# AIGC-Audio/AudioGPT

Measured on NVIDIA H100. Metric: mel_frames_per_s_vocoded, higher is better.
Workload: dtype f32

## Files before the change

audiogpt_b200/csrc/hifigan.cu:

```cuda
#include "common.cuh"
#include "tapconv.cuh"
#include "models.h"
#include "voc_kernels.cuh"

namespace agpt {

__global__ void cf_to_cl_kernel(const float* __restrict__ in, float* __restrict__ out, int C, int T) {
  __shared__ float tile[32][33];
  const int b = blockIdx.z, t0 = blockIdx.x * 32, c0 = blockIdx.y * 32;
  const float* ib = in + (long)b * C * T;
  float* ob = out + (long)b * C * T;
  for (int i = threadIdx.y; i < 32; i += blockDim.y) {
    const int c = c0 + i, t = t0 + threadIdx.x;
    tile[i][threadIdx.x] = (c < C && t < T) ? ib[(long)c * T + t] : 0.f;
  }
  __syncthreads();
  for (int i = threadIdx.y; i < 32; i += blockDim.y) {
    const int t = t0 + i, c = c0 + threadIdx.x;
    if (t < T && c < C) ob[(long)t * C + c] = tile[threadIdx.x][i];
  }
}

void launch_cf_to_cl(const float* in, float* out, int B, int C, int T, cudaStream_t st) {
  dim3 grid(cdiv(T, 32), cdiv(C, 32), B), block(32, 8);
// ... 239 lines not shown
    double inc = run;
#pragma unroll
    for (int o = 1; o < 32; o <<= 1) { const double v = __shfl_up_sync(0xffffffffu, inc, o); if (lane >= o) inc += v; }
    __syncthreads();
    if (lane == 31) wsum[warp] = inc;
    __syncthreads();
    double base = cbase[((long)b * dim + h) * nch + c];
    for (int w = 0; w < warp; ++w) base += wsum[w];
    base += inc - run;
#pragma unroll
    for (int k = 0; k < 4; ++k) {
      const int t = t0 + k;
      if (t >= L) continue;
      double ph = base + r[k];
      ph -= floor(ph);
      const float sn = sinf((float)ph * 6.283185307179586f) * sine_amp;
      const float uv = fv[k] > thr ? 1.f : 0.f;
      const float na = uv * noise_std + (1.f - uv) * sine_amp / 3.f;
      const float nz = noise ? noise[((long)b * L + t) * dim + h] : 0.f;
      acc[k] = fmaf(lin.w[h], sn * uv + na * nz, acc[k]);
    }
  }
#pragma unroll
  for (int k = 0; k < 4; ++k)
    if (t0 + k < L) har[(long)b * L + t0 + k] = tanhf(acc[k]);
}

static DevBuf g_nsf_scratch[16];

void nsf_source(const float* f0, int B, int L, int dim, float sr, const float* lin_w_host, float lin_b,
                const float* rand_ini, const float* noise, float sine_amp, float noise_std, float thr, float* har,
                cudaStream_t st) {
  AGPT_CHECK(B >= 1 && L >= 1 && dim >= 1 && dim <= NSF_MAXH, "nsf_source: bad shape (at most 16 harmonics)");
  int dev = 0;
  AGPT_CUDA(cudaGetDevice(&dev));
  const int nch = cdiv(L, NSF_CHUNK);
  double* cs = reinterpret_cast<double*>(g_nsf_scratch[dev & 15].ensure((size_t)B * dim * nch * 2 + 2));
  NsfLin lin;
  for (int h = 0; h < NSF_MAXH; ++h) lin.w[h] = h < dim ? lin_w_host[h] : 0.f;
  lin.b = lin_b;
  nsf_chunk_sum_kernel<<<dim3(nch, dim, B), 256, 0, st>>>(f0, cs, L, dim, sr);
  nsf_chunk_scan_kernel<<<cdiv(B * dim, 64), 64, 0, st>>>(cs, rand_ini, nch, dim, B);
  nsf_source_kernel<<<dim3(nch, B), 256, 0, st>>>(f0, cs, noise, har, L, dim, sr, sine_amp, noise_std, thr, lin);
  count_launch(3);
  AGPT_CUDA(cudaGetLastError());
}

struct SnakeW { DevBuf a, inv_b; };

struct ResBlockW {
  int ks = 0;
  std::vector<int> dil;
  std::vector<PackedConv> c1, c2;
  std::vector<PackedConv> c1g, c2g;
  std::vector<int> g1, g2;
  std::vector<SnakeW> act;
};

struct NoiseConvW {
  DevBuf w, b;
  int K = 0, st = 1, pad = 0, C = 0;
};

struct Hifigan : Handle {
  agpt_hifigan_cfg cfg;
  PackedConv conv_pre;
  std::vector<PackedConv> ups;
  std::vector<ResBlockW> rbs;
  std::vector<NoiseConvW> noise;
  DevBuf post_w, post_b;
  SnakeW act_post;
  AaFilter aaf;
  int c_last = 0, hop = 1;
  DevBuf melT, buf[6], sbuf;
  DevBuf plane[6];
  DevBuf io_mel, io_wav, io_har;
  float* pin_mel = nullptr; float* pin_wav = nullptr; size_t pin_mel_n = 0, pin_wav_n = 0;
  cudaStream_t own_stream = nullptr;
  bool fuse_resblock = true;
  bool tall_tiles = true;
  bool plane_feed = true;
  bool pair_dual = true;
  bool pair_pipe = true;
  bool narrow_pipe = true;
  bool conv_pipe = true;

  ~Hifigan() override {
    if (pin_mel) cudaFreeHost(pin_mel);
    if (pin_wav) cudaFreeHost(pin_wav);
    if (own_stream) cudaStreamDestroy(own_stream);
  }

  void forward(const float* mel, const float* har, int B, int T, float* wav, cudaStream_t st) {
    AGPT_CHECK(B >= 1 && T >= 1, "empty batch");
    const int C0 = cfg.upsample_initial_channel;
    size_t mx = (size_t)T * C0;
    {
      long L = T; int C = C0;
      for (int i = 0; i < cfg.num_upsamples; ++i) { L *= cfg.upsample_rates[i]; C /= 2; mx = std::max(mx, (size_t)L * C); }
    }
    mx *= (size_t)B;
    for (auto& b : buf) b.ensure(mx);
    melT.ensure((size_t)B * T * cfg.n_mels);
    float *cur = buf[0].p, *acc = buf[1].p, *X = buf[2].p, *A = buf[3].p, *R0 = buf[4].p, *R1 = buf[5].p;
    const bool big = cfg.activation != 0;
    if (big) sbuf.ensure(mx);
    float* S = sbuf.p;
    const bool planes = plane_feed && !big && tc_enabled();
    auto has_plane = [&](int ch) { return planes && ch > 128 && ch % 8 == 0; };
    size_t mxp = 0;
    {
      long Lp = T; int Cp = C0;
      for (int i = 0; i <= cfg.num_upsamples; ++i) {
        if (has_plane(Cp)) mxp = std::max(mxp, (size_t)B * Lp * Cp);
        if (i < cfg.num_upsamples) { Lp *= cfg.upsample_rates[i]; Cp /= 2; }
      }
    }
    if (mxp) for (auto& p : plane) p.ensure(mxp);
    auto plane_hi = [&](const float* t) -> __half* {
      for (int k = 0; k < 6; ++k)
        if (buf[k].p == t) return reinterpret_cast<__half*>(plane[k].p);
      throw Error("hifigan: no operand plane for this tensor");
    };
    auto feed = [&](TapConvParams& P, int ch) {
      if (!has_plane(ch)) return;
      P.pi_hi = plane_hi(P.in); P.pi_lo = P.pi_hi + mxp;
      P.tc_conv_pipe = conv_pipe;
    };
    auto emit = [&](TapConvParams& P, int ch, bool keep_fp32) {
      if (!has_plane(ch)) return;
      P.po_hi = plane_hi(P.out); P.po_lo = P.po_hi + mxp; P.po_slope = 0.1f;
      if (!keep_fp32) P.out = nullptr;
    };
    auto split = [&](const float* t, long rows, int ch) {
      if (has_plane(ch)) plane_split(t, plane_hi(t), plane_hi(t) + mxp, rows * ch, 0.1f, st);
    };
    auto snake = [&](const float* src, float* dst, long Lr, int Cr, const SnakeW& w) {
      aa_snake(src, dst, w.a.p, w.inv_b.p, aaf.f, B, (int)Lr, Cr, st);
    };
    launch_cf_to_cl(mel, melT.p, B, cfg.n_mels, T, st);
    {
      TapConvParams P = tapconv_params(conv_pre, B, T, 0, 1);
      P.in = melT.p; P.in_gstride = (long)T * cfg.n_mels; P.in_pitch = cfg.n_mels;
      P.out = cur; P.out_gstride = (long)T * C0; P.out_pitch = C0;
      P.pro = PRO_NONE; P.epi = EPI_BIAS;
      P.tc_tall = tall_tiles;
      tapconv_launch(P, st);
    }
    split(cur, (long)B * T, C0);
    long L = T; int C = C0;
    const float inv_nk = 1.f / (float)cfg.num_kernels;
    for (int i = 0; i < cfg.num_upsamples; ++i) {
      const int u = cfg.upsample_rates[i];
      const int Co = C / 2;
      {
        TapConvParams P = tapconv_params(ups[i], B, (int)L, 0, 1);
        P.in = cur; P.in_gstride = L * C; P.in_pitch = C;
        P.out = X; P.out_gstride = L * u * Co; P.out_pitch = u * Co;
        P.pro = big ? PRO_NONE : PRO_LRELU; P.slope = 0.1f; P.epi = EPI_BIAS;
        P.tc_tall = tall_tiles;
        feed(P, C);
        if (!har) emit(P, Co, true);
        tapconv_launch(P, st);
      }
      L *= u; C = Co;
      if (har) {
        AGPT_CHECK(cfg.use_nsf, "har_source given but the generator has no noise_convs");
        const NoiseConvW& nc = noise[i];
        nsf_add(X, har, nc.w.p, nc.b.p, B, (int)L, C, T * hop, nc.K, nc.st, nc.pad, st);
        split(X, (long)B * L, C);
      }
      const long gs = L * C;
      auto gview = [&](int g) { return (g && L % g == 0) ? g : 1; };
      auto conv = [&](const PackedConv& plain, const PackedConv& grouped, int gq, int dil, const float* in, float* out) {
        TapConvParams P = gq > 1 ? tapconv_params(grouped, B, (int)(L / gq), 0, 1) : tapconv_params(plain, B, (int)L, 0, dil);
        P.in = in; P.in_gstride = gs; P.in_pitch = gq * C;
        P.out = out; P.out_gstride = gs; P.out_pitch = gq * C;
        P.pro = big ? PRO_NONE : PRO_LRELU; P.slope = 0.1f;
        P.tc_tall = tall_tiles;
        return P;
      };
      for (int j = 0; j < cfg.num_kernels; ++j) {
        const ResBlockW& rb = rbs[i * cfg.num_kernels + j];
        const float* x = X;
        const int nd = (int)rb.dil.size();
        for (int n = 0; n < nd; ++n) {
          const bool last = (n == nd - 1);
          float* dst = last ? acc : ((n & 1) ? R1 : R0);
          const bool dst_plane = !last || (j == cfg.num_kernels - 1 && i + 1 < cfg.num_upsamples);
          auto residual_epi = [&](TapConvParams& P) {
            P.res = x; P.res_gstride = gs; P.res_pitch = P.in_pitch;
            if (last) { P.epi = EPI_ACC; P.scale = inv_nk; P.accumulate = (j > 0); }
            else P.epi = EPI_RES;
          };
          const bool t1 = cfg.resblock_type == 1;
          if (t1 && !big && fuse_resblock) {
            const int gq = gview(rb.g1[n]) == gview(rb.g2[n]) ? gview(rb.g1[n]) : 1;
            TapConvParams P1 = conv(rb.c1[n], rb.c1g[n], gq, rb.dil[n], x, A);
            P1.epi = EPI_BIAS;
            P1.tc_dual = pair_dual;
            P1.tc_pipe = pair_pipe;
            P1.tc_narrow_pipe = narrow_pipe;
            feed(P1, C);
            TapConvParams P2 = conv(rb.c2[n], rb.c2g[n], gq, 1, A, dst);
            residual_epi(P2);
            if (dst_plane) emit(P2, C, true);
            if (tcpair_launch(P1, P2, st)) { x = dst; continue; }
          }
          const float* conv_in = x;
          if (t1) {
            if (big) snake(x, S, L, C, rb.act[2 * n]);
            TapConvParams P = conv(rb.c1[n], rb.c1g[n], gview(rb.g1[n]), rb.dil[n], big ? S : x, A);
            P.epi = EPI_BIAS;
            feed(P, C);
            emit(P, C, false);
            tapconv_launch(P, st);
            conv_in = A;
          }
          if (big) {
            snake(conv_in, S, L, C, rb.act[t1 ? 2 * n + 1 : n]);
            conv_in = S;
          }
          TapConvParams P = t1 ? conv(rb.c2[n], rb.c2g[n], gview(rb.g2[n]), 1, conv_in, dst)
                               : conv(rb.c1[n], rb.c1g[n], gview(rb.g1[n]), rb.dil[n], conv_in, dst);
          residual_epi(P);
          feed(P, C);
          if (dst_plane) emit(P, C, true);
          tapconv_launch(P, st);
          x = dst;
        }
      }
      std::swap(cur, acc);
    }
    {
      const float* pin = cur;
      float slope = 0.01f;
      if (big) { snake(cur, S, L, C, act_post); pin = S; slope = 1.f; }
      launch_conv_post(pin, post_w.p, post_b.p, wav, B, (int)L, C, cfg.c_out, slope, st);
    }
  }
};

Handle* hifigan_create(const agpt_hifigan_cfg* cfg, const float* const* W, int nW, int device) {
  DeviceGuard dg_(device);
  const int nu = cfg->num_upsamples, nk = cfg->num_kernels;
  AGPT_CHECK(nu >= 1 && nu <= AGPT_MAX_UPS && nk >= 1 && nk <= AGPT_MAX_RBK, "bad config");
  const int C0 = cfg->upsample_initial_channel;
  for (int i = 0, C = C0; i < nu; ++i, C /= 2)
    AGPT_CHECK(C % 2 == 0 && (C / 2) % 4 == 0, "channel counts must stay multiples of 4");
  for (int j = 0; j < nk; ++j)
    AGPT_CHECK(cfg->resblock_kernel_sizes[j] % 2 == 1 && cfg->resblock_kernel_sizes[j] <= kMaxTaps,
               "resblock kernel size must be odd and <= 11");
  for (int i = 0; i < nu; ++i)
    AGPT_CHECK(cfg->upsample_rates[i] >= 1 && cfg->upsample_kernel_sizes[i] >= cfg->upsample_rates[i] &&
                   (cfg->upsample_kernel_sizes[i] - cfg->upsample_rates[i]) % 2 == 0,
               "upsample kernel size k and rate u need k >= u and an even k - u (else the stage does not output L*u samples)");
  std::unique_ptr<Hifigan> h(new Hifigan());
  h->magic = kMagicHifigan; h->device = device; h->cfg = *cfg;
  { const char* e = getenv("AGPT_FUSE_RESBLOCK"); h->fuse_resblock = !(e && e[0] == '0'); }
  { const char* e = getenv("AGPT_TALL_TILES"); h->tall_tiles = !(e && e[0] == '0'); }
  { const char* e = getenv("AGPT_PLANE_FEED"); h->plane_feed = !(e && e[0] == '0'); }
  { const char* e = getenv("AGPT_PAIR_DUAL"); h->pair_dual = !(e && e[0] == '0'); }
  { const char* e = getenv("AGPT_PAIR_PIPE"); h->pair_pipe = !(e && e[0] == '0'); }
  { const char* e = getenv("AGPT_NARROW_PIPE"); h->narrow_pipe = !(e && e[0] == '0'); }
  { const char* e = getenv("AGPT_CONV_PIPE"); h->conv_pipe = !(e && e[0] == '0'); }
  WeightCursor wc{W, nW};
  { const float* w = wc.next(); const float* b = wc.next(); pack_conv(h->conv_pre, w, b, C0, cfg->n_mels, 7, false); }
  h->ups.resize(nu);
  int C = C0; h->hop = 1;
  for (int i = 0; i < nu; ++i) {
    const float* w = wc.next(); const float* b = wc.next();
    const int u = cfg->upsample_rates[i], k = cfg->upsample_kernel_sizes[i];
    pack_convtranspose(h->ups[i], w, b, C, C / 2, k, u, (k - u) / 2);
    C /= 2; h->hop *= u;
  }
  h->c_last = C;
  auto load_snake = [&](SnakeW& sw, int ch) {
    const float* al = wc.next();
    const float* be = (cfg->activation == 2) ? wc.next() : al;
    std::vector<float> a(ch), ib(ch);
    for (int c = 0; c < ch; ++c) {
      const float av = cfg->snake_logscale ? std::exp(al[c]) : al[c];
      const float bv = cfg->snake_logscale ? std::exp(be[c]) : be[c];
      a[c] = av;
      ib[c] = 1.0f / (bv + 0.000000001f);
    }
    sw.a.upload(a); sw.inv_b.upload(ib);
  };
  h->rbs.resize((size_t)nu * nk);
  C = C0;
  for (int i = 0; i < nu; ++i) {
    C /= 2;
    for (int j = 0; j < nk; ++j) {
      ResBlockW& rb = h->rbs[i * nk + j];
      rb.ks = cfg->resblock_kernel_sizes[j];
      const int nd = cfg->resblock_num_dilations[j];
      rb.dil.assign(cfg->resblock_dilations[j], cfg->resblock_dilations[j] + nd);
      auto group_of = [&](int dil) {
        if (cfg->activation != 0 || dil != 1 || rb.ks < 7) return 0;
        if (C == 32) return 4;
        if (C == 64 && rb.ks >= 11) return 2;
        return 0;
      };
      rb.c1.resize(nd); rb.c1g.resize(nd); rb.g1.assign(nd, 0);
      for (int n = 0; n < nd; ++n) {
        const float* w = wc.next(); const float* b = wc.next();
        pack_conv(rb.c1[n], w, b, C, C, rb.ks, false);
        rb.g1[n] = group_of(rb.dil[n]);
        if (rb.g1[n]) pack_conv_grouped(rb.c1g[n], w, b, C, rb.ks, rb.g1[n]);
      }
      if (cfg->resblock_type == 1) {
        rb.c2.resize(nd); rb.c2g.resize(nd); rb.g2.assign(nd, 0);
        for (int n = 0; n < nd; ++n) {
          const float* w = wc.next(); const float* b = wc.next();
          pack_conv(rb.c2[n], w, b, C, C, rb.ks, false);
          rb.g2[n] = group_of(1);
          if (rb.g2[n]) pack_conv_grouped(rb.c2g[n], w, b, C, rb.ks, rb.g2[n]);
        }
      }
      if (cfg->activation != 0) {
        rb.act.resize(cfg->resblock_type == 1 ? 2 * nd : nd);
        for (auto& a : rb.act) load_snake(a, C);
      }
    }
  }
  if (cfg->activation != 0) load_snake(h->act_post, C);
  {
    const float* w = wc.next(); const float* b = wc.next();
    std::vector<float> pw((size_t)cfg->c_out * 7 * C);
    for (int oc = 0; oc < cfg->c_out; ++oc)
      for (int c = 0; c < C; ++c)
        for (int k = 0; k < 7; ++k) pw[((size_t)oc * 7 + k) * C + c] = w[((size_t)oc * C + c) * 7 + k];
    h->post_w.upload(pw);
    h->post_b.upload(b, cfg->c_out);
  }
  if (cfg->activation != 0) {
    const float* f = wc.next();
    for (int k = 0; k < 12; ++k) h->aaf.f[k] = f[k];
  }
  if (cfg->use_nsf) {
    wc.next(); wc.next();
    h->noise.resize(nu);
    int Cc = C0;
    for (int i = 0; i < nu; ++i) {
      Cc /= 2;
      NoiseConvW& nc = h->noise[i];
// ... 46 lines not shown
```

audiogpt_b200/csrc/tcconv5.cu:

```cuda
#include "tapconv.cuh"
#include "tapconv_epi.cuh"
#include "tc_common.cuh"
#include "tc_h16.cuh"
#include "tc_tma.cuh"
#include "models.h"

#include <set>

namespace agpt {

namespace {

constexpr int MAX_NA = 4, MAX_NW = 8;
constexpr int kMaxDyn = 227 * 1024 - 256;
constexpr int kDualDyn = 113 * 1024 - 256;

struct Tc5Smem {
  uint32_t a_hi[MAX_NA], a_lo[MAX_NA], w[MAX_NW], raw[2], rowinfo, rowp, bars, total;
};
__host__ __device__ inline void tc5_layout(Tc5Smem& s, int BN, int MT, int RRA, int NA, int NW, int NR, bool pl = false,
                                           int raw_pitch = 256) {
  uint32_t o = 0;
  for (int i = 0; i < MAX_NA; ++i) { s.a_hi[i] = o; if (i < NA) o += RRA * 128; }
  for (int i = 0; i < MAX_NA; ++i) { s.a_lo[i] = o; if (i < NA) o += RRA * 128; }
// ... 514 lines not shown
        }
        if (NR == 1 && h + 1 < nh) {
          named_bar_sync(1, NWK);
          issue_half(h + 1, 0);
        }
      }
      fence_proxy_async();
      named_bar_sync(1, NWK);
      } else {
      const uint8_t* rawb = smem + S.raw[rb];
#pragma unroll 2
      for (int idx = xt; idx < RRA * 8; idx += NWK) {
        const int row = idx >> 3, q = idx & 7;
        if (q >= nq) continue;
        const float4 x0 = pro_apply5(P1, *reinterpret_cast<const float4*>(rawb + row * 256 + q * 16), true, nullptr);
        const float4 x1 = pro_apply5(P1, *reinterpret_cast<const float4*>(rawb + row * 256 + 128 + q * 16), true, nullptr);
        uint4 h, l;
        split8(x0, x1, h, l);
        const uint32_t o = sw128(row, q);
        *reinterpret_cast<uint4*>(ahi + o) = h;
        *reinterpret_cast<uint4*>(alo + o) = l;
      }
      fence_proxy_async();
      named_bar_sync(1, NWK);
      if (c + NR < nchunks) issue_raw1(c + NR, rb);
      }
      mma_taps(P1, smem_u32(ahi) + (uint32_t)(wg * (MT / 2) - lo) * 128u, smem_u32(alo) + (uint32_t)(wg * (MT / 2) - lo) * 128u,
               (kv + 15) >> 4);
      if (NA == 1) {
        mma_drain(acc, w_empty, prev);
        prev = -1;
      }
    }
    mma_drain(acc, w_empty, prev);
    prev = -1;
    named_bar_sync(1, NWK);
    const int nch2 = P2.tc_chunks_h;
    uint8_t* a2 = smem + S.a_hi[0];
    const uint32_t lo_part = (uint32_t)nch2 * P2.R * 128;
    const int r0 = wg * (MT / 2) + (warp & 3) * 16 + (lane >> 2), c0 = 2 * (lane & 3);
    pair_handoff<MT>(acc, P1, P2, a2, nch2, P2.R, Lv, r0, c0, qa, xt, NWK);
    named_bar_sync(1, NWK);
    for (int c = 0; c < nch2; ++c) {
      const uint32_t ahi0 = smem_u32(a2) + (uint32_t)c * P2.R * 128 + (uint32_t)(wg * (MT / 2) - P2.lo_al) * 128u;
      mma_taps(P2, ahi0, ahi0 + lo_part, (min(H_KCH, P2.Cin - c * H_KCH) + 15) >> 4);
    }
    tile_epilogue<BN, MT, HALF ? 1 : 4, false>(acc, P2, g, 0, rowp, smem, S, wg, xt);
  } else if (lane == 0) {
    const uint32_t bytes = 2u * BN * 128u;
    const int total2 = P2.tc_chunks_h * P2.ntaps;
    for (int it = 0; it < total + total2; ++it) {
      const uint8_t* src = it < total ? reinterpret_cast<const uint8_t*>(P1.w_h) + (size_t)it * bytes
                                      : reinterpret_cast<const uint8_t*>(P2.w_h) + (size_t)(it - total) * bytes;
      ring_put(smem, S.w, w_full, w_empty, NW, it, src, bytes);
    }
  }
}

template <int BN, int MT>
__global__ void __launch_bounds__(V5_THREADS, 1) tcpair_kernel(const __grid_constant__ TapConvParams P1,
                                                               const __grid_constant__ TapConvParams P2) {
  tcpair_body<BN, MT>(P1, P2);
}
template <int BN>
__global__ void __launch_bounds__(V5_THREADS, 2) tcpair2_kernel(const __grid_constant__ TapConvParams P1,
                                                                const __grid_constant__ TapConvParams P2) {
  tcpair_body<BN, TC_ROWS, true>(P1, P2);
}

constexpr int PIPE_THREADS = 512;
constexpr uint32_t PIPE_STAGE = 2u * 128u * 64u;
__device__ __forceinline__ uint64_t make_desc64(uint32_t saddr) {
  uint64_t d = 0;
  d |= (uint64_t)((saddr & 0x3FFFF) >> 4);
  d |= (uint64_t)1 << 16;
  d |= (uint64_t)(512 >> 4) << 32;
  d |= (uint64_t)2 << 62;
  return d;
}
constexpr int PIPE_MMA = 256, PIPE_DATA = 128;
template <int N> __device__ __forceinline__ void setmaxnreg_inc() { asm volatile("setmaxnreg.inc.sync.aligned.u32 %0;" ::"n"(N)); }
template <int N> __device__ __forceinline__ void setmaxnreg_dec() { asm volatile("setmaxnreg.dec.sync.aligned.u32 %0;" ::"n"(N)); }

constexpr int PIPE_MAX_NW = 8;
struct PipeSmem { uint32_t set[2], w[PIPE_MAX_NW], bars, total; };
__host__ __device__ inline void pipe_layout(PipeSmem& s, int R1, int NW) {
  uint32_t o = 0;
  for (int i = 0; i < 2; ++i) { s.set[i] = o; o += (uint32_t)R1 * 512; }
  for (int i = 0; i < PIPE_MAX_NW; ++i) { s.w[i] = o; if (i < NW) o += PIPE_STAGE; }
  s.bars = o; o += (2 * PIPE_MAX_NW + 4) * 8;
  s.total = o;
}

__global__ void __launch_bounds__(PIPE_THREADS, 1) tcpair_pipe_kernel(const __grid_constant__ TapConvParams P1,
                                                                      const __grid_constant__ TapConvParams P2) {
  constexpr int BN = 128, MT = TC_ROWS;
  extern __shared__ uint8_t smem_raw_[];
  uint8_t* smem = reinterpret_cast<uint8_t*>((reinterpret_cast<uintptr_t>(smem_raw_) + 1023) & ~(uintptr_t)1023);
  const int R1 = P1.R, NW = P1.tc_nw;
  __shared__ PipeSmem S;
  if (threadIdx.x == 0) pipe_layout(S, R1, NW);
  __syncthreads();
  uint64_t* w_full = reinterpret_cast<uint64_t*>(smem + S.bars);
  uint64_t* w_empty = w_full + PIPE_MAX_NW;
  uint64_t* in_full = w_full + 2 * PIPE_MAX_NW;
  uint64_t* acc_full = in_full + 2;

  const int tid = threadIdx.x, warp = tid >> 5, lane = tid & 31;
  const int wg = __shfl_sync(0xffffffffu, tid >> 7, 0);
  int span2 = 0;
  for (int t = 0; t < P2.ntaps; ++t) span2 = max(span2, P2.tap_off[t] - P2.lo_al);
  const int Lv = P1.L, MTO = MT - span2, ntx = (Lv + MTO - 1) / MTO, ntiles = ntx * P1.G;
  const int nloc = (int)blockIdx.x < ntiles ? (ntiles - 1 - (int)blockIdx.x) / (int)gridDim.x + 1 : 0;
  const int lo = P1.lo_al, nch = P1.tc_chunks_h, total1 = 2 * nch * P1.ntaps;
  const int RR2 = P2.R, nch2 = P2.tc_chunks_h, total2 = 2 * nch2 * P2.ntaps;
  auto tile_of = [&](int k, int& g, int& q0) {
    const int T = (int)blockIdx.x + k * (int)gridDim.x;
    g = T / ntx;
    q0 = (T - g * ntx) * MTO;
  };

  if (tid == 0) {
    for (int i = 0; i < NW; ++i) { mbar_init(&w_full[i], 1); mbar_init(&w_empty[i], PIPE_MMA / 32); }
    for (int i = 0; i < 2; ++i) { mbar_init(&in_full[i], PIPE_DATA); mbar_init(&acc_full[i], PIPE_MMA); }
    fence_barrier_init();
  }
  __syncthreads();

  if (wg < 2) {
    setmaxnreg_inc<168>();
    float acc[1][1][BN / 2];
    int it = 0, prev = -1;
    auto mma_taps = [&](const TapConvParams& Q, uint32_t ahi0, uint32_t alo0) {
      for (int t = 0; t < Q.ntaps; ++t)
        for (int hf = 0; hf < 2; ++hf, ++it) {
          const int s = it % NW;
          mbar_wait(&w_full[s], (uint32_t)((it / NW) & 1));
          const uint32_t shift = (uint32_t)Q.tap_off[t] * 128u;
          const uint64_t dah = make_desc(ahi0 + shift) + 4 * hf, dal = make_desc(alo0 + shift) + 4 * hf;
          const uint32_t ws = smem_u32(smem + S.w[s]);
          fence_tile(acc);
          wgmma_fence();
#pragma unroll
          for (int k = 0; k < 2; ++k) {
            const uint64_t ko = (uint64_t)((k * 32) >> 4);
            const uint64_t dwh = make_desc64(ws) + ko, dwl = make_desc64(ws + BN * 64) + ko;
            wgmma_n128(acc[0][0], dah + ko, dwh);
            wgmma_n128(acc[0][0], dal + ko, dwh);
            wgmma_n128(acc[0][0], dah + ko, dwl);
          }
          wgmma_commit();
          wgmma_wait<1>();
          fence_tile(acc);
          if (prev >= 0 && lane == 0) mbar_arrive(&w_empty[prev]);
          prev = s;
        }
    };
    const int r0 = wg * (MT / 2) + (warp & 3) * 16 + (lane >> 2), c0 = 2 * (lane & 3);
    for (int k = 0; k < nloc; ++k) {
      int g, q0;
      tile_of(k, g, q0);
      const int qa = q0 + P2.lo_al;
      uint8_t* set = smem + S.set[k & 1];
      zero_tile(acc);
      mbar_wait(&in_full[k & 1], (uint32_t)((k >> 1) & 1));
      for (int c = 0; c < nch; ++c) {
        const uint32_t ahi0 = smem_u32(set) + (uint32_t)c * R1 * 128 + (uint32_t)(wg * (MT / 2) - lo) * 128u;
        mma_taps(P1, ahi0, ahi0 + (uint32_t)nch * R1 * 128);
      }
      mma_drain(acc, w_empty, prev);
      prev = -1;
      named_bar_sync(1, PIPE_MMA);
      pair_handoff<MT>(acc, P1, P2, set, nch2, RR2, Lv, r0, c0, qa, tid, PIPE_MMA);
      named_bar_sync(1, PIPE_MMA);
      const uint32_t lo_part = (uint32_t)nch2 * RR2 * 128;
      for (int c = 0; c < nch2; ++c) {
        const uint32_t ahi0 = smem_u32(set) + (uint32_t)c * RR2 * 128 + (uint32_t)(wg * (MT / 2) - P2.lo_al) * 128u;
        mma_taps(P2, ahi0, ahi0 + lo_part);
      }
      mma_drain(acc, w_empty, prev);
      prev = -1;
      named_bar_sync(1, PIPE_MMA);
#pragma unroll
      for (int blk = 0; blk < BN / 32; ++blk) stage_block(acc, set + blk * (MT * 128), blk * 32, r0, c0, P2.tc_descale);
      mbar_arrive(&acc_full[k & 1]);
    }
  } else if (wg == 2) {
    setmaxnreg_inc<152>();
    const int dt = tid - PIPE_MMA;
    auto transform = [&](int k) {
      int g, q0;
      tile_of(k, g, q0);
      const int rin = q0 + P2.lo_al + lo;
      const float* __restrict__ ing = P1.in + g * P1.in_gstride;
      uint8_t* set = smem + S.set[k & 1];
      const int items = R1 * nch * 8;
#pragma unroll 4
      for (int idx = dt; idx < items; idx += PIPE_DATA) {
        const int row = idx / (nch * 8), c = (idx >> 3) % nch, q = idx & 7;
        const int r = rin + row, ch = c * H_KCH + 8 * q;
        float4 v0 = make_float4(0.f, 0.f, 0.f, 0.f), v1 = v0;
        if (r >= 0 && r < Lv && ch < P1.Cin) {
          v0 = ldg_stream(ing + (long)r * P1.in_pitch + ch);
          v1 = ldg_stream(ing + (long)r * P1.in_pitch + ch + 4);
        }
        const float4 x0 = pro_apply5(P1, v0, true, nullptr), x1 = pro_apply5(P1, v1, true, nullptr);
        uint4 h, l;
        split8(x0, x1, h, l);
        const uint32_t o = (uint32_t)c * R1 * 128 + sw128(row, q);
        *reinterpret_cast<uint4*>(set + o) = h;
        *reinterpret_cast<uint4*>(set + (uint32_t)nch * R1 * 128 + o) = l;
      }
      fence_proxy_async();
      mbar_arrive(&in_full[k & 1]);
    };
    auto epilogue = [&](int k) {
      int g, q0;
      tile_of(k, g, q0);
      const uint8_t* set = smem + S.set[k & 1];
      const int jc = dt & 7;
      for (int blk = 0; blk < BN / 32; ++blk) {
        const int cb = blk * 32;
        const uint8_t* stg = set + blk * (MT * 128);
        const float4 cv = epi_colvec(P2, g, cb + 4 * jc);
        for (int h = 0; h < 2; ++h) {
          EpiPre pre[4];
          int pp[4];
#pragma unroll
          for (int i = 0; i < 4; ++i) {
            const int row = (dt + (4 * h + i) * PIPE_DATA) >> 3;
            pp[i] = (row < MTO && q0 + row < Lv) ? q0 + row : -1;
            if (pp[i] >= 0) epi_load(P2, g, pp[i], cb + 4 * jc, pre[i]);
          }
#pragma unroll
          for (int i = 0; i < 4; ++i) {
            const int row = (dt + (4 * h + i) * PIPE_DATA) >> 3;
            if (pp[i] >= 0)
              epi_store_cv(P2, g, pp[i], cb + 4 * jc, *reinterpret_cast<const float4*>(stg + sw128(row, jc)), pre[i], cv);
          }
        }
      }
    };
    if (nloc > 0) transform(0);
    for (int k = 0; k < nloc; ++k) {
      if (k + 1 < nloc) transform(k + 1);
      mbar_wait(&acc_full[k & 1], (uint32_t)((k >> 1) & 1));
      epilogue(k);
      named_bar_sync(2, PIPE_DATA);
    }
  } else {
    setmaxnreg_dec<24>();
    if (warp != 12 || lane != 0) return;
    int n_it = 0;
    for (int k = 0; k < nloc; ++k)
      for (int it = 0; it < total1 + total2; ++it, ++n_it) {
        const uint8_t* src = it < total1 ? reinterpret_cast<const uint8_t*>(P1.w_hk) + (size_t)it * PIPE_STAGE
                                         : reinterpret_cast<const uint8_t*>(P2.w_hk) + (size_t)(it - total1) * PIPE_STAGE;
        ring_put(smem, S.w, w_full, w_empty, NW, n_it, src, PIPE_STAGE);
      }
  }
}

constexpr int NARROW_THREADS = 640;
constexpr int NARROW_MMA = 256, NARROW_DATA = 128, NARROW_WG = 128;
constexpr int NARROW_MMA_REGS = 112, NARROW_XF_REGS = 80, NARROW_EPI_REGS = 152;
constexpr int NARROW_MAX_NS = 4, NARROW_MAX_NW = 22;
struct NarrowSmem { uint32_t op[NARROW_MAX_NS], raw[NARROW_MAX_NS], w[NARROW_MAX_NW], bars, total; };
__host__ __device__ inline void narrow_layout(NarrowSmem& s, int BN, int R1, int nbox, int NS, int NW) {
  uint32_t o = 0;
  for (int i = 0; i < NARROW_MAX_NS; ++i) { s.op[i] = o; if (i < NS) o += (uint32_t)R1 * 256; }
  for (int i = 0; i < NARROW_MAX_NS; ++i) { s.raw[i] = o; if (i < NS) o += (uint32_t)R1 * 128 * nbox; }
  for (int i = 0; i < NARROW_MAX_NW; ++i) { s.w[i] = o; if (i < NW) o += 2u * BN * 128; }
  s.bars = o; o += (2 * NARROW_MAX_NW + 4 * NARROW_MAX_NS) * 8;
  s.total = o;
}

template <int BN>
__global__ void __launch_bounds__(NARROW_THREADS, 1) tcpair_narrow_kernel(const __grid_constant__ TapConvParams P1,
                                                                          const __grid_constant__ TapConvParams P2,
                                                                          const __grid_constant__ CUtensorMap tmx) {
  constexpr int NB = tc5_nb(BN), MT = TC_ROWS;
  static_assert(NB == BN && BN <= 64, "narrow pairs: one wgmma column block");
  extern __shared__ uint8_t smem_raw_[];
  uint8_t* smem = reinterpret_cast<uint8_t*>((reinterpret_cast<uintptr_t>(smem_raw_) + 1023) & ~(uintptr_t)1023);
  const int R1 = P1.R, NS = P1.tc_na, NW = P1.tc_nw, nbox = (P1.Cin + 31) >> 5;
  __shared__ NarrowSmem S;
  if (threadIdx.x == 0) narrow_layout(S, BN, R1, nbox, NS, NW);
  __syncthreads();
  uint64_t* w_full = reinterpret_cast<uint64_t*>(smem + S.bars);
  uint64_t* w_empty = w_full + NARROW_MAX_NW;
  uint64_t* raw_full = w_empty + NARROW_MAX_NW;
  uint64_t* in_full = raw_full + NARROW_MAX_NS;
  uint64_t* acc_full = in_full + NARROW_MAX_NS;
  uint64_t* set_free = acc_full + NARROW_MAX_NS;

  const int tid = threadIdx.x, warp = tid >> 5, lane = tid & 31;
  const int wg = __shfl_sync(0xffffffffu, tid >> 7, 0);
  int span2 = 0;
  for (int t = 0; t < P2.ntaps; ++t) span2 = max(span2, P2.tap_off[t] - P2.lo_al);
  const int Lv = P1.L, MTO = MT - span2, ntx = (Lv + MTO - 1) / MTO, ntiles = ntx * P1.G;
  const int nloc = (int)blockIdx.x < ntiles ? (ntiles - 1 - (int)blockIdx.x) / (int)gridDim.x + 1 : 0;
  const int lo = P1.lo_al, RR2 = P2.R;
  const int total1 = P1.ntaps, iters = total1 + P2.ntaps;
  const bool wres = NW == iters;
  auto tile_of = [&](int k, int& g, int& q0) {
    const int T = (int)blockIdx.x + k * (int)gridDim.x;
    g = T / ntx;
    q0 = (T - g * ntx) * MTO;
  };

  if (tid == 0) {
    for (int i = 0; i < NW; ++i) { mbar_init(&w_full[i], 1); mbar_init(&w_empty[i], NARROW_MMA / 32); }
    for (int i = 0; i < NS; ++i) {
      mbar_init(&raw_full[i], 1);
      mbar_init(&in_full[i], NARROW_DATA);
      mbar_init(&acc_full[i], NARROW_WG);
      mbar_init(&set_free[i], NARROW_DATA);
    }
    fence_barrier_init();
  }
  __syncthreads();

  if (wg < 2) {
    setmaxnreg_inc<NARROW_MMA_REGS>();
    float acc[2][1][BN / 2];
    int it = 0, prev = -1;
    auto mma_taps = [&](const TapConvParams& Q, uint32_t ahi0, uint32_t alo0, int ksteps) {
      for (int t = 0; t < Q.ntaps; ++t, ++it) {
        const int s = it % NW;
        mbar_wait(&w_full[s], wres ? 0u : (uint32_t)((it / NW) & 1));
        const uint32_t shift = (uint32_t)Q.tap_off[t] * 128u;
        mma_group(acc, make_desc(ahi0 + shift), make_desc(alo0 + shift), smem_u32(smem + S.w[s]), ksteps,
                  w_empty, wres ? -1 : prev);
        prev = s;
      }
// ... 545 lines not shown
  AGPT_CHECK(tma_encode_rows_h(&m.hi, P.pi_hi, P.Cin, P.L, P.G, P.in_pitch, P.in_gstride, br) &&
                 tma_encode_rows_h(&m.lo, P.pi_lo, P.Cin, P.L, P.G, P.in_pitch, P.in_gstride, br),
             "cannot encode the operand-plane tensor maps");
  return m;
}

static bool tcconv5_try(TapConvParams P, int BN, int MT, cudaStream_t st) {
  tc5_rows(P, MT);
  size_t smem = 0;
  if (!tc5_plan(P, BN, MT, 0, P.tc_chunks_h * P.ntaps, smem)) return false;
  const int Lv = tc_lv(P);
  dim3 grid(cdiv(Lv, MT), cdiv(P.Cout, BN), tc_groups(P));
  tapconv_note_launch(1, BN, MT, P.pi_hi ? 1 : 0, AGPT_TC_KERN_TILE);
  if (P.pi_hi) {
    const PlMaps m = pl_tensor_maps(P);
    tc_launch(tcconv5_pl_kern(BN, MT), false, grid, dim3(V5_THREADS), smem, st, P, m.hi, m.lo);
  } else {
    tc_launch(tcconv5_kern(BN, MT), false, grid, dim3(V5_THREADS), smem, st, P);
  }
  if (MT == TC_TALL) profile_count_tall();
  if (P.pi_hi) profile_count_plane();
  return true;
}

HTile pick_h_tile(const TapConvParams& P, int sms) {
  const int Lv = tc_lv(P);
  const long rt = (long)cdiv(Lv, TC_ROWS) * tc_groups(P);
  auto cost = [](int bn) { return bn == 128 ? 1.0 : (bn == 96 ? 0.82 : (bn == 64 ? 0.62 : 0.45)); };
  HTile best{P.tc_bn, P.w_h, rt * cdiv(P.Cout, P.tc_bn), TC_ROWS};
  double bs = (double)cdiv(best.ntiles, (long)sms) * cost(P.tc_bn);
  auto consider = [&](int bn, const float* w) {
    if (!w) return;
    const long nt = rt * cdiv(P.Cout, bn);
    const double sc = (double)cdiv(nt, (long)sms) * cost(bn);
    if (sc < bs - 1e-9) { bs = sc; best = HTile{bn, w, nt, TC_ROWS}; }
  };
  if (P.tc_bn == 128) consider(64, P.w_h64);
  if (P.tc_bn == 128) consider(96, P.w_h96);
  const long tall = (long)cdiv(Lv, TC_TALL) * tc_groups(P) * cdiv(P.Cout, best.bn);
  if (tc5_tall(P, best.bn, tall, sms)) { best.mt = TC_TALL; best.ntiles = tall; }
  return best;
}

static bool tcpair_try(TapConvParams P1, TapConvParams P2, int MT, bool dual, cudaStream_t st) {
  const int BN = P1.tc_bn;
  tc5_rows(P1, MT);
  const int span2 = tc5_rows(P2, MT);
  P2.tc_bn = BN;
  size_t smem = 0;
  const long a2bytes = 2L * P2.tc_chunks_h * P2.R * 128;
  const int iters = P1.tc_chunks_h * P1.ntaps + P2.tc_chunks_h * P2.ntaps;
  if (dual ? !tcpair_plan_dual(P1, BN, a2bytes, iters, smem) : !tc5_plan(P1, BN, MT, a2bytes, iters, smem)) return false;
  dim3 grid(cdiv(tc_lv(P1), MT - span2), 1, tc_groups(P1));
  const auto dual_kern = BN == 64 ? tcpair2_kernel<64> : tcpair2_kernel<32>;
  if (dual) {
    tc_func_attrs(reinterpret_cast<const void*>(dual_kern), true);
    int per_sm = 0;
    AGPT_CUDA(cudaOccupancyMaxActiveBlocksPerMultiprocessor(&per_sm, dual_kern, V5_THREADS, smem));
    if (per_sm != 2) return false;
  }
  void* rec = profile_begin_pair(P1, P2, st);
  tapconv_note_launch(1, BN, MT, 0, dual ? AGPT_TC_KERN_DUAL : AGPT_TC_KERN_TILE);
  if (dual) {
    tc_launch(dual_kern, true, grid, dim3(V5_THREADS), smem, st, P1, P2);
    profile_count_dual();
  } else {
    tc_launch(tcpair_kern(BN, MT), false, grid, dim3(V5_THREADS), smem, st, P1, P2);
    if (MT == TC_TALL) profile_count_tall();
  }
  profile_end(rec, st);
  count_launch(1);
  AGPT_CUDA(cudaGetLastError());
  return true;
}

static bool tcpair_pipe_try(TapConvParams P1, TapConvParams P2, cudaStream_t st) {
  if (!P1.tc_pipe || P1.tc_bn != 128 || P1.Cin != 128 || P1.Cout != 128 || P2.Cout != 128 || !P1.w_hk || !P2.w_hk)
    return false;
  tc5_rows(P1, TC_ROWS);
  const int span2 = tc5_rows(P2, TC_ROWS);
  if (P2.R > P1.R) return false;
  const long wbytes = PIPE_STAGE;
  PipeSmem S;
  pipe_layout(S, P1.R, 0);
  const long spare = (long)kMaxDyn - 1024 - (long)S.total;
  if (spare < 4 * wbytes) return false;
  const int iters = 2 * (P1.tc_chunks_h * P1.ntaps + P2.tc_chunks_h * P2.ntaps);
  P1.tc_nw = (int)std::min<long>(std::min<long>(PIPE_MAX_NW, iters), spare / wbytes);
  P2.tc_bn = 128;
  pipe_layout(S, P1.R, P1.tc_nw);
  const size_t smem = (size_t)S.total + 1024;
  const long tiles = (long)cdiv(P1.L, TC_ROWS - span2) * P1.G;
  dim3 grid((unsigned)std::min<long>(tiles, tc5_sms()));
  void* rec = profile_begin_pair(P1, P2, st);
  tapconv_note_launch(1, 128, TC_ROWS, 0, AGPT_TC_KERN_PAIR_PIPE);
  tc_launch(tcpair_pipe_kernel, false, grid, dim3(PIPE_THREADS), smem, st, P1, P2);
  profile_count_pipe();
  profile_end(rec, st);
  count_launch(1);
  AGPT_CUDA(cudaGetLastError());
  return true;
}

static bool tcpair_dual(const TapConvParams& P1) {
  return P1.tc_dual && P1.tc_bn <= 64;
}

static bool tcpair_narrow_try(TapConvParams P1, TapConvParams P2, cudaStream_t st) {
  const int BN = P1.tc_bn, iters = P1.ntaps + P2.ntaps;
  if (!P1.tc_narrow_pipe || (BN != 64 && BN != 32) || (BN == 64 && iters > 14) || P1.Cin > BN ||
      P2.res != P1.in || P2.res_pitch != P1.in_pitch || P2.res_gstride != P1.in_gstride)
    return false;
  const int span1 = tc5_rows(P1, TC_ROWS);
  const int span2 = tc5_rows(P2, TC_ROWS);
  if (P2.R > P1.R || P1.R > 256 || P1.lo_al > 0 || P2.lo_al > 0 || (P1.lo_al + span1) + (P2.lo_al + span2) < 0)
    return false;
  const int nbox = cdiv(P1.Cin, 32);
  const long wbytes = 2L * BN * 128, set = 256L * P1.R + 128L * nbox * P1.R;
  NarrowSmem S;
  narrow_layout(S, BN, P1.R, nbox, 0, 0);
  const long avail = (long)kMaxDyn - 1024 - (long)S.total;
  int NS = 2, NW;
  if (avail - iters * wbytes >= 2 * set) {
    NW = iters;
    NS = (int)std::min<long>(NARROW_MAX_NS, (avail - iters * wbytes) / set);
  } else {
    NW = (int)std::min<long>(iters, (avail - NS * set) / wbytes);
    if (NW < 2) return false;
  }
  CUtensorMap tmx;
  if (!tma_encode_rows(&tmx, P1.in, P1.Cin, P1.L, P1.G, P1.in_pitch, P1.in_gstride, P1.R)) return false;
  P1.tc_na = NS; P1.tc_nw = NW;
  P2.tc_bn = BN;
  narrow_layout(S, BN, P1.R, nbox, NS, NW);
  const size_t smem = (size_t)S.total + 1024;
  const long tiles = (long)cdiv(P1.L, TC_ROWS - span2) * P1.G;
  dim3 grid((unsigned)std::min<long>(tiles, tc5_sms()));
  void* rec = profile_begin_pair(P1, P2, st);
  tapconv_note_launch(1, BN, TC_ROWS, 0, AGPT_TC_KERN_NARROW_PIPE);
  tc_launch(BN == 64 ? tcpair_narrow_kernel<64> : tcpair_narrow_kernel<32>, false, grid, dim3(NARROW_THREADS), smem, st, P1,
            P2, tmx);
  profile_count_dual();
  profile_count_narrow_pipe();
  profile_end(rec, st);
  count_launch(1);
  AGPT_CUDA(cudaGetLastError());
  return true;
}

bool tcpair_launch(TapConvParams P1, TapConvParams P2, cudaStream_t st) {
  if (!tcconv_supported(P1) || !P2.w_h) return false;
  const int BN = P1.tc_bn;
  if (P1.pi_hi || P2.po_hi) return false;
  if (P2.tc_bn != BN || P1.Cout > BN || P2.Cin != P1.Cout || P2.Cout > BN || P1.Wreal || P2.Wreal || P1.strips ||
      P1.G != P2.G || P1.L != P2.L || P1.pro != PRO_LRELU || P2.pro != PRO_LRELU || (P2.epi != EPI_RES && P2.epi != EPI_ACC))
    return false;
  if (tcpair_pipe_try(P1, P2, st)) return true;
  if (tcpair_dual(P1) && (tcpair_narrow_try(P1, P2, st) || tcpair_try(P1, P2, TC_ROWS, true, st))) return true;
  const int span2 = tc5_rows(P2, TC_TALL);
  if (tc5_tall(P1, BN, (long)cdiv(tc_lv(P1), TC_TALL - span2) * tc_groups(P1), tc5_sms()) &&
      tcpair_try(P1, P2, TC_TALL, false, st))
    return true;
  return tcpair_try(P1, P2, TC_ROWS, false, st);
}

static bool tcconv_pipe_try(TapConvParams P, const HTile& c, cudaStream_t st) {
  if (!P.tc_conv_pipe || !P.pi_hi || P.Wreal || P.strips || c.bn != 128 || c.mt != TC_ROWS ||
      (P.epi != EPI_BIAS && P.epi != EPI_RES && P.epi != EPI_ACC))
    return false;
  P.w_h = c.w;
  P.tc_bn = 128;
  tc5_rows(P, TC_ROWS);
  const int PR = pl_rows(P.R);
  const long abytes = 256L * PR, wbytes = 2L * 128 * 128;
  CpipeSmem S;
  cpipe_layout(S, PR, 0, 0);
  const long avail = (long)kMaxDyn - 1024 - (long)S.total;
  int NA = std::min(MAX_NA, std::max(2, P.tc_chunks_h));
  while (NA > 2 && NA * abytes + 3 * wbytes > avail) --NA;
// ... 28 lines not shown
```

Measured before the change: 208,900.

## Add TMA-staged variant of paired resblock pipe kernel with separate transform and epilogue warpgroups

Adds a templated staged version of the fused conv-pair pipe kernel. In it, TMA warps load raw input tiles and residual boxes into shared memory, a dedicated warpgroup converts them to split hi/lo operands in place, and a separate epilogue warpgroup reads residuals from smem slots, including ones reused from the dead tail of the input set. The goal is to take global residual and input loads off the epilogue's critical path and overlap transform, MMA and epilogue across tiles. It costs more threads, more mbarrier handshakes and lower register budgets per role, and it falls back to the old kernel when the residual is not the input or TMA encoding fails.

```diff
diff --git a/audiogpt_b200/csrc/hifigan.cu b/audiogpt_b200/csrc/hifigan.cu
--- a/audiogpt_b200/csrc/hifigan.cu
+++ b/audiogpt_b200/csrc/hifigan.cu
@@ -345,6 +345,7 @@
   bool plane_feed = true;
   bool pair_dual = true;
   bool pair_pipe = true;
+  bool pair_pipe_stage = true;
   bool narrow_pipe = true;
   bool conv_pipe = true;
 
@@ -462,7 +463,7 @@
             TapConvParams P1 = conv(rb.c1[n], rb.c1g[n], gq, rb.dil[n], x, A);
             P1.epi = EPI_BIAS;
             P1.tc_dual = pair_dual;
-            P1.tc_pipe = pair_pipe;
+            P1.tc_pipe = pair_pipe ? (pair_pipe_stage ? 1 : 2) : 0;
             P1.tc_narrow_pipe = narrow_pipe;
             feed(P1, C);
             TapConvParams P2 = conv(rb.c2[n], rb.c2g[n], gq, 1, A, dst);
@@ -525,6 +526,7 @@
   { const char* e = getenv("AGPT_PLANE_FEED"); h->plane_feed = !(e && e[0] == '0'); }
   { const char* e = getenv("AGPT_PAIR_DUAL"); h->pair_dual = !(e && e[0] == '0'); }
   { const char* e = getenv("AGPT_PAIR_PIPE"); h->pair_pipe = !(e && e[0] == '0'); }
+  { const char* e = getenv("AGPT_PAIR_PIPE_STAGE"); h->pair_pipe_stage = !(e && e[0] == '0'); }
   { const char* e = getenv("AGPT_NARROW_PIPE"); h->narrow_pipe = !(e && e[0] == '0'); }
   { const char* e = getenv("AGPT_CONV_PIPE"); h->conv_pipe = !(e && e[0] == '0'); }
   WeightCursor wc{W, nW};
diff --git a/audiogpt_b200/csrc/tcconv5.cu b/audiogpt_b200/csrc/tcconv5.cu
--- a/audiogpt_b200/csrc/tcconv5.cu
+++ b/audiogpt_b200/csrc/tcconv5.cu
@@ -620,29 +620,38 @@
 template <int N> __device__ __forceinline__ void setmaxnreg_inc() { asm volatile("setmaxnreg.inc.sync.aligned.u32 %0;" ::"n"(N)); }
 template <int N> __device__ __forceinline__ void setmaxnreg_dec() { asm volatile("setmaxnreg.dec.sync.aligned.u32 %0;" ::"n"(N)); }
 
-constexpr int PIPE_MAX_NW = 8;
-struct PipeSmem { uint32_t set[2], w[PIPE_MAX_NW], bars, total; };
-__host__ __device__ inline void pipe_layout(PipeSmem& s, int R1, int NW) {
+constexpr int PIPE_MAX_NW = 8, PIPE_MAX_RES = 8;
+constexpr uint32_t PIPE_RES_BOX = 32u * 128u, PIPE_DUMP = 128u * 512u;
+struct PipeSmem { uint32_t set[2], w[PIPE_MAX_NW], res[PIPE_MAX_RES], bars, total; };
+__host__ __device__ inline void pipe_layout(PipeSmem& s, int R1, int NW, int NSP) {
   uint32_t o = 0;
   for (int i = 0; i < 2; ++i) { s.set[i] = o; o += (uint32_t)R1 * 512; }
   for (int i = 0; i < PIPE_MAX_NW; ++i) { s.w[i] = o; if (i < NW) o += PIPE_STAGE; }
-  s.bars = o; o += (2 * PIPE_MAX_NW + 4) * 8;
+  for (int i = 0; i < PIPE_MAX_RES; ++i) { s.res[i] = o; if (i < NSP) o += PIPE_RES_BOX; }
+  s.bars = o; o += (2 * PIPE_MAX_NW + 8 + 2 * PIPE_MAX_RES) * 8;
   s.total = o;
 }
-
-__global__ void __launch_bounds__(PIPE_THREADS, 1) tcpair_pipe_kernel(const __grid_constant__ TapConvParams P1,
-                                                                      const __grid_constant__ TapConvParams P2) {
+constexpr int PIPE_STAGED_THREADS = 640, PIPE_XF_REGS = 48, PIPE_EPI_REGS = 72;
+
+template <bool STAGED>
+__global__ void __launch_bounds__(STAGED ? PIPE_STAGED_THREADS : PIPE_THREADS, 1)
+    tcpair_pipe_kernel(const __grid_constant__ TapConvParams P1, const __grid_constant__ TapConvParams P2,
+                       const __grid_constant__ CUtensorMap tmx, const __grid_constant__ CUtensorMap tmr) {
   constexpr int BN = 128, MT = TC_ROWS;
   extern __shared__ uint8_t smem_raw_[];
   uint8_t* smem = reinterpret_cast<uint8_t*>((reinterpret_cast<uintptr_t>(smem_raw_) + 1023) & ~(uintptr_t)1023);
-  const int R1 = P1.R, NW = P1.tc_nw;
+  const int R1 = P1.R, NW = P1.tc_nw, NSP = P1.tc_na;
   __shared__ PipeSmem S;
-  if (threadIdx.x == 0) pipe_layout(S, R1, NW);
+  if (threadIdx.x == 0) pipe_layout(S, R1, NW, NSP);
   __syncthreads();
   uint64_t* w_full = reinterpret_cast<uint64_t*>(smem + S.bars);
   uint64_t* w_empty = w_full + PIPE_MAX_NW;
   uint64_t* in_full = w_full + 2 * PIPE_MAX_NW;
   uint64_t* acc_full = in_full + 2;
+  uint64_t* raw_full = acc_full + 2;
+  uint64_t* set_free = raw_full + 2;
+  uint64_t* res_full = set_free + 2;
+  uint64_t* res_empty = res_full + PIPE_MAX_RES;
 
   const int tid = threadIdx.x, warp = tid >> 5, lane = tid & 31;
   const int wg = __shfl_sync(0xffffffffu, tid >> 7, 0);
@@ -658,9 +667,18 @@
     q0 = (T - g * ntx) * MTO;
   };
 
+  const int NSL = (R1 - 128) / 8, NRS = NSP + NSL, nj = (MTO + 31) / 32, NU = 4 * nj;
+  auto res_slot = [&](int j, int s) -> uint8_t* {
+    return j < NSP ? smem + S.res[j] : smem + S.set[s] + PIPE_DUMP + (uint32_t)(j - NSP) * PIPE_RES_BOX;
+  };
+
   if (tid == 0) {
     for (int i = 0; i < NW; ++i) { mbar_init(&w_full[i], 1); mbar_init(&w_empty[i], PIPE_MMA / 32); }
     for (int i = 0; i < 2; ++i) { mbar_init(&in_full[i], PIPE_DATA); mbar_init(&acc_full[i], PIPE_MMA); }
+    if constexpr (STAGED) {
+      for (int i = 0; i < 2; ++i) { mbar_init(&raw_full[i], 1); mbar_init(&set_free[i], PIPE_DATA); }
+      for (int i = 0; i < NRS; ++i) { mbar_init(&res_full[i], 1); mbar_init(&res_empty[i], PIPE_DATA); }
+    }
     fence_barrier_init();
   }
   __syncthreads();
@@ -723,7 +741,71 @@
       for (int blk = 0; blk < BN / 32; ++blk) stage_block(acc, set + blk * (MT * 128), blk * 32, r0, c0, P2.tc_descale);
       mbar_arrive(&acc_full[k & 1]);
     }
-  } else if (wg == 2) {
+  } else if (STAGED && wg == 2) {
+    setmaxnreg_dec<PIPE_XF_REGS>();
+    const int dt = tid - PIPE_MMA, i16 = dt & 15, c = i16 >> 3, q = i16 & 7, odd = q >> 2;
+    const uint32_t qsz = (uint32_t)R1 * 128, src = (uint32_t)(2 * c + odd) * qsz;
+    for (int k = 0; k < nloc; ++k) {
+      const int s = k & 1;
+      mbar_wait(&raw_full[s], (uint32_t)((k >> 1) & 1));
+      uint8_t* set = smem + S.set[s];
+      for (int row = dt >> 4; row < R1; row += PIPE_DATA / 16) {
+        const uint8_t* rr = set + src + row * 128;
+        const int u0 = 2 * (q & 3), sw = row & 7;
+        const float4 a = *reinterpret_cast<const float4*>(rr + (((u0 + odd) ^ sw) << 4));
+        const float4 b = *reinterpret_cast<const float4*>(rr + (((u0 + 1 - odd) ^ sw) << 4));
+        __syncwarp();
+        const float4 x0 = pro_apply5(P1, odd ? b : a, true, nullptr), x1 = pro_apply5(P1, odd ? a : b, true, nullptr);
+        uint4 h, l;
+        split8(x0, x1, h, l);
+        const uint32_t o = (uint32_t)c * qsz + sw128(row, q);
+        *reinterpret_cast<uint4*>(set + o) = h;
+        *reinterpret_cast<uint4*>(set + 2 * qsz + o) = l;
+      }
+      fence_proxy_async();
+      mbar_arrive(&in_full[s]);
+    }
+  } else if (STAGED && wg == 3) {
+    setmaxnreg_dec<PIPE_EPI_REGS>();
+    const int dt = tid - PIPE_MMA - PIPE_DATA, jc = dt & 7;
+    int n = 0;
+    for (int k = 0; k < nloc; ++k) {
+      int g, q0;
+      tile_of(k, g, q0);
+      const int s = k & 1;
+      const uint8_t* set = smem + S.set[s];
+      mbar_wait(&acc_full[s], (uint32_t)((k >> 1) & 1));
+      for (int b = 0; b < 4; ++b) {
+        const int co = 32 * b + 4 * jc;
+        const uint8_t* stg = set + b * (MT * 128);
+        const float4 cv = epi_colvec(P2, g, co);
+        for (int j = 0; j < nj; ++j, ++n) {
+          float4 ob[2];
+          int pp[2];
+#pragma unroll
+          for (int i = 0; i < 2; ++i) {
+            const int row = 32 * j + (dt >> 3) + 16 * i;
+            pp[i] = (row < MTO && q0 + row < Lv) ? q0 + row : -1;
+            ob[i] = pp[i] >= 0 ? epi_load_b(P2, g, pp[i], co) : make_float4(0.f, 0.f, 0.f, 0.f);
+          }
+          const int slot = n % NRS;
+          mbar_wait(&res_full[slot], (uint32_t)((n / NRS) & 1));
+          const uint8_t* rb = res_slot(slot, s);
+#pragma unroll
+          for (int i = 0; i < 2; ++i) {
+            const int rl = (dt >> 3) + 16 * i, row = 32 * j + rl;
+            EpiPre pre;
+            pre.a = *reinterpret_cast<const float4*>(rb + sw128(rl, jc));
+            pre.b = ob[i];
+            if (pp[i] >= 0) epi_store_cv(P2, g, pp[i], co, *reinterpret_cast<const float4*>(stg + sw128(row, jc)), pre, cv);
+          }
+          mbar_arrive(&res_empty[slot]);
+        }
+      }
+      fence_proxy_async();
+      mbar_arrive(&set_free[s]);
+    }
+  } else if (!STAGED && wg == 2) {
     setmaxnreg_inc<152>();
     const int dt = tid - PIPE_MMA;
     auto transform = [&](int k) {
@@ -788,7 +870,43 @@
     }
   } else {
     setmaxnreg_dec<24>();
-    if (warp != 12 || lane != 0) return;
+    constexpr int wwarp = STAGED ? 16 : 12;
+    if (lane != 0) return;
+    if (STAGED && warp == wwarp + 1) {
+      tma_prefetch_desc(&tmx);
+      for (int k = 0; k < nloc; ++k) {
+        int g, q0;
+        tile_of(k, g, q0);
+        const int s = k & 1;
+        if (k >= 2) mbar_wait(&set_free[s], (uint32_t)(((k >> 1) - 1) & 1));
+        mbar_arrive_expect_tx(&raw_full[s], 4u * R1 * 128u);
+        for (int b = 0; b < 4; ++b)
+          tma_load_3d(smem + S.set[s] + (uint32_t)b * R1 * 128, &tmx, 32 * b, q0 + P2.lo_al + lo, g, &raw_full[s]);
+      }
+      return;
+    }
+    if (STAGED && warp == wwarp + 2) {
+      tma_prefetch_desc(&tmr);
+      int n = 0;
+      for (int k = 0; k < nloc; ++k) {
+        int g, q0;
+        tile_of(k, g, q0);
+        const int s = k & 1;
+        bool c2_done = false;
+        for (int u = 0; u < NU; ++u, ++n) {
+          const int slot = n % NRS;
+          if (n >= NRS) mbar_wait(&res_empty[slot], (uint32_t)((n / NRS - 1) & 1));
+          if (slot >= NSP && !c2_done) {
+            mbar_wait(&acc_full[s], (uint32_t)((k >> 1) & 1));
+            c2_done = true;
+          }
+          mbar_arrive_expect_tx(&res_full[slot], PIPE_RES_BOX);
+          tma_load_3d(res_slot(slot, s), &tmr, 32 * (u / nj), q0 + 32 * (u % nj), g, &res_full[slot]);
+        }
+      }
+      return;
+    }
+    if (warp != wwarp) return;
     int n_it = 0;
     for (int k = 0; k < nloc; ++k)
       for (int it = 0; it < total1 + total2; ++it, ++n_it) {
@@ -1500,19 +1618,30 @@
   if (P2.R > P1.R) return false;
   const long wbytes = PIPE_STAGE;
   PipeSmem S;
-  pipe_layout(S, P1.R, 0);
+  pipe_layout(S, P1.R, 0, 0);
   const long spare = (long)kMaxDyn - 1024 - (long)S.total;
   if (spare < 4 * wbytes) return false;
   const int iters = 2 * (P1.tc_chunks_h * P1.ntaps + P2.tc_chunks_h * P2.ntaps);
   P1.tc_nw = (int)std::min<long>(std::min<long>(PIPE_MAX_NW, iters), spare / wbytes);
+  const int nsl = (P1.R - 128) / 8;
+  const int nsp = (int)std::min<long>(PIPE_MAX_RES - nsl, (spare - P1.tc_nw * wbytes) / PIPE_RES_BOX);
+  CUtensorMap tmx{}, tmr{};
+  const bool staged = P1.tc_pipe == 1 && P2.res == P1.in && P2.res_pitch == P1.in_pitch &&
+                      P2.res_gstride == P1.in_gstride && nsl + nsp >= 1 &&
+                      tma_encode_rows(&tmx, P1.in, 128, P1.L, P1.G, P1.in_pitch, P1.in_gstride, P1.R) &&
+                      tma_encode_rows(&tmr, P1.in, 128, P1.L, P1.G, P1.in_pitch, P1.in_gstride, 32);
+  P1.tc_na = staged ? nsp : 0;
   P2.tc_bn = 128;
-  pipe_layout(S, P1.R, P1.tc_nw);
+  pipe_layout(S, P1.R, P1.tc_nw, P1.tc_na);
   const size_t smem = (size_t)S.total + 1024;
   const long tiles = (long)cdiv(P1.L, TC_ROWS - span2) * P1.G;
   dim3 grid((unsigned)std::min<long>(tiles, tc5_sms()));
   void* rec = profile_begin_pair(P1, P2, st);
   tapconv_note_launch(1, 128, TC_ROWS, 0, AGPT_TC_KERN_PAIR_PIPE);
-  tc_launch(tcpair_pipe_kernel, false, grid, dim3(PIPE_THREADS), smem, st, P1, P2);
+  if (staged)
+    tc_launch(tcpair_pipe_kernel<true>, false, grid, dim3(PIPE_STAGED_THREADS), smem, st, P1, P2, tmx, tmr);
+  else
+    tc_launch(tcpair_pipe_kernel<false>, false, grid, dim3(PIPE_THREADS), smem, st, P1, P2, tmx, tmr);
   profile_count_pipe();
   profile_end(rec, st);
   count_launch(1);
```

Result: faster. 215,600 (median of 6 runs) (+3.2%).
